# ndpp/ndpp

Hardware: AMD Instinct MI355X
Metric: E_in points*Legendre-orders/sec (free-gas scatter moments) (higher is better)
Workload: dtype f64

## Files before the change

ndpp_amd/csrc/fg_device.h:

```cpp
#pragma once

#include <hip/hip_runtime.h>

#include "fg_pipeline.h"

namespace ndpp {
namespace {

constexpr int kWave = 64;
constexpr int kMuWavesPerSimd = 2;
constexpr int kMuBlocksPerCU = 4 * kMuWavesPerSimd;

struct DevAtomics {
  __device__ static int add(int* p, int v) { return atomicAdd(p, v); }
};

typedef __attribute__((address_space(3))) double lds_f64;
typedef __attribute__((address_space(3))) unsigned lds_u32;

constexpr int mu_stack_fields(int R) { return 2 + 2 * R; }
constexpr int mu_lds_levels(int R) {
  const int budget = (160 * 1024) / kMuBlocksPerCU - 64;
  const int fit = budget / (kWave * (8 * mu_stack_fields(R) + 4));
  return (R == 1 && fit > kStackLdsLevels) ? kStackLdsLevels : fit;
// ... 38 lines not shown
        Xb[r] = lds[o + (2 + r) * kWave];
        Xe[r] = lds[o + (2 + R + r) * kWave];
      }
      m = ldsm[(d - d0) * kWave + lane];
    } else {
      const double* p = (const double*)(gbase + (size_t)(goff + __umul24((unsigned)d, gstride)));
      b = p[0]; w = p[1];
#pragma unroll
      for (int r = 0; r < R; ++r) { Xb[r] = p[2 + r]; Xe[r] = p[2 + R + r]; }
      m = *(const unsigned*)(p + NF);
    }
  }
};

__global__ void fg_prep_kernel(FgBatch B, int level) {
  if (*B.overflow) return;
  const int base = B.lvl_off(level);
  const int nt = B.n_tasks(level);
  for (int t = blockIdx.x * blockDim.x + threadIdx.x; t < nt;
       t += gridDim.x * blockDim.x)
    fg_prep_task(B, level, base, t);
}

template <int R, int LMAX, bool kPath>
__device__ __forceinline__ void mu_wave_loop(const FgBatch& B, int level, int base, int nt,
                                             int* counter, DevMuStack<R>& st) {
  MuLane<R, LMAX> s;
  s.mask = 0;
  const PnConsts pk = make_pn_consts<(R * LMAX <= 12 && LMAX <= 8)>();
  bool active = false, more = true;
  bool counts = true;
  unsigned long long n_k = 0, n_v = 0, n_i = 0, n_o = 0;
  unsigned long long w_it = 0, l_it = 0;
  const int kTaskBlock = nt >= (int)(gridDim.x * 16 * kWave) ? 4 * kWave : kWave;
  int blk_next = 0, blk_end = 0;
  constexpr int kFetchMin = kPath ? 8 : 1;
  auto lanes = [](bool x) -> unsigned long long { return __builtin_amdgcn_ballot_w64(x); };
  for (;;) {
    unsigned long long need = more ? lanes(!active) : 0ull;
    if (kFetchMin > 1 && need && __popcll(need) < kFetchMin && lanes(active)) need = 0;
    if (need) {
      if (blk_next >= blk_end) {
        const int first = __ffsll((long long)need) - 1;
        int b = 0;
        if (threadIdx.x == (unsigned)first) b = atomicAdd(counter, kTaskBlock);
        b = __builtin_amdgcn_readlane(b, first);
        blk_next = b;
        blk_end = (b + kTaskBlock < nt) ? b + kTaskBlock : nt;
        if (b >= nt) more = false;
      }
      if (!active && more) {
        const int rank = __popcll(need & ((1ull << threadIdx.x) - 1ull));
        const int t = blk_next + rank;
        if (t < blk_end) {
          if (kPath) mu_init_split<R, LMAX>(B, level, base, t, s);
          else mu_init<R, LMAX>(B, level, base, t, s);
          active = (s.mask != 0);
          if (kPath) counts = (s.path_bits == 0);
          if (active) mu_tot_zero(s);
        }
      }
      const int taken = __popcll(need);
      blk_next = (blk_next + taken < blk_end) ? blk_next + taken : blk_end;
    }
    const unsigned long long act = lanes(active);
    if (!act && !more) break;
    w_it += 1;
    l_it += (unsigned long long)__popcll(act);
    if (active) {
      if (!mu_step<R, LMAX, DevMuStack<R>, kPath>(B, s, st, pk)) {
        mu_finish(B, s, kPath);
        n_k += 2ull * s.visits + 3;
        n_v += s.visits;
        n_o += s.ovisits;
        n_i += counts ? 1 : 0;
        active = false;
      }
    }
  }
// ... 8 lines not shown
    atomicAdd(&B.stats[kStatMuVisits], n_v);
    atomicAdd(&B.stats[kStatMuIntegrals], n_i);
    atomicAdd(&B.stats[kStatOrderVisits], n_o);
    atomicAdd(&B.stats[kStatWaveIters], w_it);
    atomicAdd(&B.stats[kStatLaneIters], l_it);
  }
}

template <int R, int LMAX>
__global__ __launch_bounds__(kWave, kMuWavesPerSimd) void fg_mu_kernel(FgBatch B, int level, double* gstack, int* counter) {
  constexpr int NF = mu_stack_fields(R), kLevels = mu_lds_levels(R);
  __shared__ double lds[kLevels * NF * kWave];
  __shared__ unsigned ldsm[kLevels * kWave];
  DevMuStack<R> st;
  st.lds = (lds_f64*)lds;
  st.ldsm = (lds_u32*)ldsm;
  st.gbase = (char*)gstack;
  st.goff = (blockIdx.x * kWave + threadIdx.x) * DevMuStack<R>::kRecBytes;
  st.gstride = gridDim.x * kWave * DevMuStack<R>::kRecBytes;
  st.lane = threadIdx.x;
  st.d0 = B.mu_its > kLevels ? B.mu_its - kLevels : 0;

  if (*B.overflow) return;
  const int base = B.lvl_off(level);
  if (B.split_level(level))
    mu_wave_loop<R, LMAX, true>(B, level, base, B.n_mu_tasks(level) * kSplit, counter, st);
  else
    mu_wave_loop<R, LMAX, false>(B, level, base, B.n_mu_tasks(level), counter, st);
}

__global__ void fg_seg_zero_kernel(FgBatch B, int level) {
  if (*B.overflow || !B.split_level(level)) return;
  const size_t n = (size_t)B.n_mu_tasks(level) * kSplit * B.nch();
  for (size_t k = blockIdx.x * (size_t)blockDim.x + threadIdx.x; k < n; k += (size_t)gridDim.x * blockDim.x)
    B.seg[k] = 0.0;
}

__global__ void fg_mu_combine_kernel(FgBatch B, int level) {
  if (*B.overflow || !B.split_level(level)) return;
  const int base = B.lvl_off(level);
  const int nch = B.nch();
  const long tot = (long)B.n_mu_tasks(level) * nch;
  for (long k = blockIdx.x * (long)blockDim.x + threadIdx.x; k < tot; k += (long)gridDim.x * blockDim.x) {
    const int t = (int)(k / nch), ch = (int)(k - (long)t * nch);
    int n, slot;
    fg_task_decode(B, level, base, t, n, slot);
    const unsigned mask = (unsigned)B.node_info[4 * n + 0];
    const int r = ch / B.L, l = ch - r * B.L;
    if (!(mask & chan_bit(r, l))) continue;
    const unsigned gl_rows = B.t_gl ? B.t_gl[B.rec_index(level, base, n, slot)] : 0u;
    if (gl_rows >> r & 1u) continue;
// ... 28 lines not shown
  const int nn = B.lvl_cnt[level];
  for (int i = blockIdx.x * blockDim.x + threadIdx.x; i < nn;
       i += gridDim.x * blockDim.x)
    fg_reduce_node(B, base, i);
}

__global__ void fg_assemble_kernel(FgBatch B) {
  if (*B.overflow) return;
  const int n_calls = B.n_jobs * B.R;
  for (int c = blockIdx.x * blockDim.x + threadIdx.x; c < n_calls;
       c += gridDim.x * blockDim.x)
    fg_assemble_call(B, c);
}

inline int fg_blocks(long n, int threads = 256) {
  long b = (n + threads - 1) / threads;
  return (int)(b < 1 ? 1 : (b > 4096 ? 4096 : b));
}
inline void launch_fg_setup(const FgBatch& B, hipStream_t s) {
  hipLaunchKernelGGL(fg_setup_kernel, dim3(fg_blocks((long)B.n_jobs * B.G)), dim3(256), 0, s, B);
}
inline void launch_fg_prep(const FgBatch& B, int level, hipStream_t s) {
  hipLaunchKernelGGL(fg_prep_kernel, dim3(2048), dim3(256), 0, s, B, level);
}
inline void launch_fg_seg_zero(const FgBatch& B, int level, hipStream_t s) {
  hipLaunchKernelGGL(fg_seg_zero_kernel, dim3(4096), dim3(256), 0, s, B, level);
}
inline void launch_fg_combine(const FgBatch& B, int level, hipStream_t s) {
  hipLaunchKernelGGL(fg_mu_combine_kernel, dim3(2048), dim3(256), 0, s, B, level);
}
inline void launch_fg_node(const FgBatch& B, int level, hipStream_t s) {
  hipLaunchKernelGGL(fg_node_kernel, dim3(2048), dim3(256), 0, s, B, level);
}
inline void launch_fg_reduce(const FgBatch& B, int level, hipStream_t s) {
  hipLaunchKernelGGL(fg_reduce_kernel, dim3(2048), dim3(256), 0, s, B, level);
}
inline void launch_fg_assemble(const FgBatch& B, hipStream_t s) {
  hipLaunchKernelGGL(fg_assemble_kernel, dim3(fg_blocks((long)B.n_jobs * B.R)), dim3(256), 0, s, B);
}

#if NDPP_FAST
template <int R, int LMAX>
__global__ __launch_bounds__(256) void fg_gauss_kernel(FgBatch B, int level) {
  __shared__ int queue[256 / kWave][2 * kWave];
  if (*B.overflow) return;
  const int base = B.lvl_off(level);
// ... 184 lines not shown
```

ndpp_amd/csrc/fg_pipeline.h:

```cpp
#pragma once

#include "ndpp_math.h"

namespace ndpp {
#if NDPP_FAST
inline namespace fast_arith {
#else
inline namespace strict_arith {
#endif

#if NDPP_FAST
constexpr int kMuBlock = 2;
#else
constexpr int kMuBlock = 1;
#endif
constexpr int kSegPerGroup = 5;
constexpr int kMaxLevels = 32;
constexpr int kStackLdsLevels = 8;
constexpr int kMaxRows = 2;
constexpr int kSplitLog2 = 4;
constexpr int kSplit = 1 << kSplitLog2;
constexpr int kRowBits = 16;

enum { kStatKEvals = 0, kStatMuVisits, kStatMuIntegrals, kStatEoutNodes,
       kStatWaveIters, kStatLaneIters, kStatOrderVisits, kStatGaussIntegrals, kNumStats };

NDPP_HD unsigned chan_bit(int r, int l) { return 1u << (r * kRowBits + l); }

struct FgBatch {
  int n_jobs, R, G, L, M;
  double A, kT;
  const double* job_A = nullptr;
  const double* job_kT = nullptr;
  const double* job_ein;
  const int* job_row;
  const double* f_tab;
  const double* e_bins;
  double sab_threshold, brent_thresh, mu_tol, eout_tol;
  int mu_its, eout_its;
  MuGrid grid;
  int ncap;
  double* node_a;
  double* node_b;
  double* node_F;
  double* node_S;
// ... 1 lines not shown
  int tcap;
  double* t_mulo;
  double* t_muhi;
  double* t_X;
  unsigned char* t_gl = nullptr;
  double gl_ratio = 2.0;
  int gl_near = 1;
  double gl_amin = 2.0E-6;
  int gl_cert_depth = 7;
  int gl_cert_depth_near = 8;
  int gl_panels = 16;
  int gl_graded = 8;
  int* lvl_cnt;
  int* next_task;
  int* overflow;
  unsigned long long* stats;
  double* seg = nullptr;
  int split_below = 0;
  const int* order = nullptr;
  const int* mask_rank = nullptr;
  const int* mu_nodes = nullptr;
  double* raw;
  int* t_alias = nullptr;

  NDPP_HD double A_of(int job) const { return job_A ? job_A[job] : A; }
  NDPP_HD double kT_of(int job) const { return job_kT ? job_kT[job] : kT; }
  NDPP_HD int nch() const { return R * L; }
  NDPP_HD int n_trees() const { return n_jobs * G * kSegPerGroup; }
  NDPP_HD int lvl_off(int level) const {
    int o = 0;
    for (int k = 0; k < level; ++k) o += lvl_cnt[k];
    return o;
  }
  NDPP_HD bool split_level(int level) const {
    const int nt = n_mu_tasks(level);
    return seg != nullptr && nt > 0 && nt <= split_below;
  }
  NDPP_HD int tasks_per_node(int level) const { return level == 0 ? 5 : 2; }
  NDPP_HD int n_tasks(int level) const { return lvl_cnt[level] * tasks_per_node(level); }
  NDPP_HD int n_mu_tasks(int level) const {
    return (mu_nodes ? *mu_nodes : lvl_cnt[level]) * tasks_per_node(level);
  }
  NDPP_HD int rec_index(int level, int base, int n, int slot) const {
    return level == 0 ? 5 * n + slot : 2 * (n - base) + (slot == 3 ? 1 : 0);
  }
  NDPP_HD double& F(int slot, int ch, int n) const {
    return node_F[((size_t)(slot * R * L + ch)) * ncap + n];
  }
  NDPP_HD double& S(int ch, int n) const { return node_S[(size_t)ch * ncap + n]; }
  NDPP_HD double& tX(int k, int r, int t) const { return t_X[((size_t)(k * R + r)) * tcap + t]; }
  NDPP_HD unsigned full_mask() const {
    unsigned m = 0;
    for (int r = 0; r < R; ++r) m |= ((1u << L) - 1u) << (r * kRowBits);
    return m;
  }
  NDPP_HD int alias_of(int level, int rec) const { return (level == 0 && t_alias && t_gl) ? t_alias[rec] : -1; }
  NDPP_HD int node_job(int n) const { return node_info[4 * n + 2] & 0x3ffffff; }
  NDPP_HD int node_depth(int n) const { return node_info[4 * n + 2] >> 26; }
};

NDPP_HD void fg_group_layout(const FgBatch& B, int job, int g, double* sa, double* sb, bool* live) {
  const double Ein = B.job_ein[job];
  const double A = B.A_of(job), kT = B.kT_of(job);
  double alphaEin = (A - 1.0) / (A + 1.0);
  alphaEin = alphaEin * alphaEin * Ein;
  double Eout_lo, Eout_hi;
  fg_eout_bounds(A, kT, Ein, Eout_lo, Eout_hi);
  const double eg = B.e_bins[g], eg1 = B.e_bins[g + 1];

  bool on[kSegPerGroup] = {false, false, false, false, false};
  if ((eg < Eout_hi) && (eg1 > Eout_lo)) {
    double Elo = (Eout_lo > eg) ? Eout_lo : eg;
    double Ehi = (Eout_hi < eg1) ? Eout_hi : eg1;
// ... 511 lines not shown
  }
  NDPP_HD void pop(int d, double& b_, double& w_, double* Xb_, double* Xe_, unsigned& m_) const {
    b_ = b[d]; w_ = w[d]; m_ = m[d];
    for (int r = 0; r < R; ++r) { Xb_[r] = Xb[d][r]; Xe_[r] = Xe[d][r]; }
  }
};

NDPP_HD int highest_bit(unsigned x) {
#if defined(__HIP_DEVICE_COMPILE__)
  return 31 - __clz((int)x);
#else
  return 31 - __builtin_clz(x);
#endif
}

NDPP_HD int popcount32(unsigned x) {
#if defined(__HIP_DEVICE_COMPILE__)
  return __popc(x);
#else
  return __builtin_popcount(x);
#endif
}

template <int R, int LMAX>
NDPP_HD void mu_init(const FgBatch& B, int level, int base, int t, MuLane<R, LMAX>& s) {
  int n, slot;
  fg_task_decode(B, level, base, t, n, slot);
  s.node = n;
  s.slot = slot;
  s.mask = (unsigned)B.node_info[4 * n + 0] & MuLane<R, LMAX>::kChanMask;
  s.pending = 0;
  s.depth = 0;
  s.visits = 0;
  s.ovisits = 0;
#pragma unroll
  for (int ch = 0; ch < R * LMAX; ++ch) s.acc[ch] = 0.0;
  s.path_left = 0; s.own_from = 0; s.path_bits = 0; s.own_pending = false; s.slot_path = 0;
  s.task = t;
  s.chans = s.mask;
  if (s.mask == 0) return;
  const int rec = B.rec_index(level, base, n, slot);
  if (B.t_gl) {
    const unsigned rows = B.t_gl[rec];
#pragma unroll
    for (int r = 0; r < R; ++r)
      if (rows >> r & 1u) s.mask &= ~(((1u << kRowBits) - 1u) << (r * kRowBits));
    s.chans = s.mask;
    if (s.mask == 0) return;
  }
  const int job = B.node_job(n);
  const double Ein = B.job_ein[job];
  const double Eout = fg_slot_point(B.node_a[n], B.node_b[n], slot);
  s.q = make_pair(B.A_of(job), B.kT_of(job), Ein, Eout);
  s.f.off = 8u * (unsigned)B.M * (unsigned)B.job_row[(size_t)job * R];
  s.a = B.t_mulo[rec];
  s.b = B.t_muhi[rec];
  double Xa[R];
#pragma unroll
  for (int r = 0; r < R; ++r) {
    Xa[r] = B.tX(0, r, rec);
    s.Xb[r] = B.tX(1, r, rec);
    s.Xc[r] = B.tX(2, r, rec);
  }
  const double h = s.b - s.a;
  s.wp = h / 6.0;
  double Pa[LMAX];
  pn_all<LMAX>(s.a, Pa, make_pn_consts());
#pragma unroll
  for (int r = 0; r < R; ++r)
#pragma unroll
    for (int l = 0; l < LMAX; ++l) s.fa[r * LMAX + l] = Xa[r] * Pa[l];
}

template <int R, int LMAX, class Stack, bool kPath = true>
NDPP_HD bool mu_step(const FgBatch& B, MuLane<R, LMAX>& s, Stack& st, const PnConsts& pk) {
  if (kPath && s.own_pending && s.depth == s.own_from) {
    s.own_pending = false;
#pragma unroll
    for (int ch = 0; ch < R * LMAX; ++ch) s.acc[ch] = 0.0;
    mu_tot_zero(s);
  }
  const double c = 0.5 * (s.a + s.b);
  const double h = s.b - s.a;
  const double d = 0.5 * (s.a + c);
  const double e = 0.5 * (c + s.b);
// ... 183 lines not shown
    s.depth = dj + 1;
    return true;
  }
  return false;
}

template <int R, int LMAX>
NDPP_HD void mu_finish(const FgBatch& B, const MuLane<R, LMAX>& s, bool split = false) {
  const unsigned mask = s.chans;
#pragma unroll
  for (int r = 0; r < R; ++r)
#pragma unroll
    for (int l = 0; l < LMAX; ++l)
      if (mask & chan_bit(r, l)) {
        if (split) {
          if (!s.own_pending)
            B.seg[((size_t)s.task * kSplit + s.slot_path) * B.nch() + r * B.L + l] = s.acc[r * LMAX + l];
          continue;
        }
        B.F(s.slot, r * B.L + l, s.node) = s.tot[r * LMAX + l] + s.acc[r * LMAX + l];
      }
}

template <int R, int LMAX>
NDPP_HD void mu_init_split(const FgBatch& B, int level, int base, int t, MuLane<R, LMAX>& s) {
  const int nt = B.n_mu_tasks(level);
  const int i = t % nt, rank = t / nt;
  mu_init<R, LMAX>(B, level, base, i, s);
  int jp = 0;
  if (s.mask != 0) {
#if NDPP_FAST
    const double pa = s.q.p, qa = s.q.q;
#else
    const double pa = s.q.EpE / s.q.AkT, qa = 2.0 * s.q.s2 / s.q.AkT;
#endif
    const double x = ((pa - fabs(s.q.beta)) / qa - s.a) / (s.b - s.a) * (double)kSplit;
    jp = (x > 0.0) ? (x < (double)(kSplit - 1) ? (int)x : kSplit - 1) : 0;
  }
  int lo = jp - 1, hi = jp, cur = hi;
  for (int k = 0; k <= rank; ++k) {
    if (((k & 1) == 0 && hi < kSplit) || lo < 0) cur = hi++;
    else cur = lo--;
  }
  s.path_left = kSplitLog2;
  s.path_bits = (unsigned)cur;
  s.slot_path = 0;
  int tz = 0;
  while (tz < kSplitLog2 && !(((unsigned)cur >> tz) & 1u)) ++tz;
  s.own_from = kSplitLog2 - tz;
  s.own_pending = (s.own_from != 0);
}

NDPP_HD void fg_mu_combine_task(const FgBatch& B, int level, int base, int t) {
  int n, slot;
  fg_task_decode(B, level, base, t, n, slot);
  const unsigned mask = (unsigned)B.node_info[4 * n + 0];
  if (mask == 0) return;
  const unsigned gl_rows = B.t_gl ? B.t_gl[B.rec_index(level, base, n, slot)] : 0u;
  const int nch = B.nch();
  for (int r = 0; r < B.R; ++r)
    for (int l = 0; l < B.L; ++l)
      if ((mask & chan_bit(r, l)) && !(gl_rows >> r & 1u)) {
        const int ch = r * B.L + l;
        double tot = 0.0;
        for (int j = 0; j < kSplit; ++j) tot = tot + B.seg[((size_t)t * kSplit + j) * nch + ch];
        B.F(slot, ch, n) = tot;
      }
}

struct HostAtomics {
  static int add(int* p, int v) { int o = *p; *p += v; return o; }
};

// ... 108 lines not shown
```

ndpp_amd/csrc/fg_strict_stages.hip:

```cpp
#include <cstring>

#include "../../include/ndpp_hip.h"
#include "fg_device.h"
#include "kernels.h"

#if NDPP_FAST
#error "fg_strict_stages.hip must be compiled with -DNDPP_FAST=0 -ffp-contract=off"
#endif

namespace ndpp {
namespace {

template <class Launch>
int strict_stage(const void* batch, size_t batch_bytes, Launch launch) {
  FgBatch B;
  if (batch_bytes != sizeof(FgBatch)) return fail(NDPP_EDEVICE, "strict stage: batch layout mismatch");
  memcpy(&B, batch, sizeof B);
  launch(B);
  return NDPP_OK;
}

int launch_fg_setup_strict(const void* batch, size_t batch_bytes, hipStream_t s) {
  return strict_stage(batch, batch_bytes, [&](const FgBatch& B) { launch_fg_setup(B, s); });
}
int launch_fg_prep_strict(const void* batch, size_t batch_bytes, int level, hipStream_t s) {
  return strict_stage(batch, batch_bytes, [&](const FgBatch& B) { launch_fg_prep(B, level, s); });
}
int launch_fg_seg_zero_strict(const void* batch, size_t batch_bytes, int level, hipStream_t s) {
  return strict_stage(batch, batch_bytes, [&](const FgBatch& B) { launch_fg_seg_zero(B, level, s); });
}
int launch_fg_mu_strict(const void* batch, size_t batch_bytes, int level, int num_cu,
                        double* gstack, int* counter, hipStream_t s) {
  return strict_stage(batch, batch_bytes,
                      [&](const FgBatch& B) { launch_mu_any(B, level, num_cu, gstack, counter, s); });
}
int launch_fg_combine_strict(const void* batch, size_t batch_bytes, int level, hipStream_t s) {
  return strict_stage(batch, batch_bytes, [&](const FgBatch& B) { launch_fg_combine(B, level, s); });
}
int launch_fg_node_strict(const void* batch, size_t batch_bytes, int level, hipStream_t s) {
  return strict_stage(batch, batch_bytes, [&](const FgBatch& B) { launch_fg_node(B, level, s); });
}
int launch_fg_reduce_strict(const void* batch, size_t batch_bytes, int level, hipStream_t s) {
  return strict_stage(batch, batch_bytes, [&](const FgBatch& B) { launch_fg_reduce(B, level, s); });
}
int launch_fg_assemble_strict(const void* batch, size_t batch_bytes, hipStream_t s) {
  return strict_stage(batch, batch_bytes, [&](const FgBatch& B) { launch_fg_assemble(B, s); });
}

}

const FgStages& fg_strict_stages() {
  static const FgStages table = {launch_fg_setup_strict,  launch_fg_prep_strict,    launch_fg_seg_zero_strict,
                                 launch_fg_mu_strict,     launch_fg_combine_strict, launch_fg_node_strict,
                                 launch_fg_reduce_strict, launch_fg_assemble_strict};
  return table;
}

}
```

ndpp_amd/csrc/kernels.h:

```cpp
#pragma once
#include <hip/hip_runtime.h>

#include <type_traits>

#include "../../include/ndpp_hip.h"

namespace ndpp {

int fail(int code, const char* fmt, ...);

#define NDPP_TRY(expr)                                                        \
  do {                                                                        \
    hipError_t e_ = (expr);                                                   \
    if (e_ != hipSuccess)                                                     \
      return fail(NDPP_EDEVICE, "%s failed: %s (%s:%d)", #expr,               \
                  hipGetErrorString(e_), __FILE__, __LINE__);                 \
  } while (0)

int require_device(const char* who = nullptr);
int check_row_lo(int n_ein, const int* row_lo, int n_rows);
int check_law9_edata(int n_edata, const double* edata);
enum ParamChecks { kCheckOrder = 1, kCheckTab = 2, kCheckFreegas = 4 };
int check_params(const ndpp_params* p, int G, int what, int n_tab = 0);

// ... 24 lines not shown

enum ProfileFamily { kProfFreegasMu = 0, kProfFreegasOther, kProfFile4, kProfFile6Cm, kProfFile6Lab,
                     kProfLaw9, kProfSab, kProfChi, kProfConvert, kNumProfileFamilies };
void profile_add(int family, double ms);
struct GpuSpan {
  hipEvent_t e0 = nullptr, e1 = nullptr;
  hipStream_t s;
  int family;
  explicit GpuSpan(hipStream_t stream = nullptr, int family = -1);
  void end();
  ~GpuSpan();
};

void launch_file4_any(int n, const int* list, int mu_bins, const double* ein,
                      const int* row_lo, const double* w_hi, const double* f_tab,
                      double awr, double Q, int G, int L, const double* e_bins,
                      int rows_per_ein, double* out, hipStream_t s,
                      const int* nuc_of_ein = nullptr, const double* nuc_awr = nullptr,
                      const double* nuc_Q = nullptr);

struct FgStages {
  int (*setup)(const void* batch, size_t bytes, hipStream_t s);
  int (*prep)(const void* batch, size_t bytes, int level, hipStream_t s);
  int (*seg_zero)(const void* batch, size_t bytes, int level, hipStream_t s);
  int (*mu)(const void* batch, size_t bytes, int level, int num_cu, double* gstack, int* counter, hipStream_t s);
  int (*combine)(const void* batch, size_t bytes, int level, hipStream_t s);
  int (*node)(const void* batch, size_t bytes, int level, hipStream_t s);
  int (*reduce)(const void* batch, size_t bytes, int level, hipStream_t s);
  int (*assemble)(const void* batch, size_t bytes, hipStream_t s);
};
const FgStages& fg_strict_stages();

struct DeviceSink {
  virtual ~DeviceSink() = default;
  virtual int consume(const double* out_d, int n, size_t GL) = 0;
};
int elastic_leg_batch_sink(const ndpp_params* p, double A, double kT, double freegas_cutoff, double Q,
                           int n_ein, const double* ein, const int* row_lo, const double* w_hi,
                           int n_rows, const double* f_tab, int G, const double* e_bins, double* out,
                           int* status, DeviceSink* sink);
int file6_batch_sink(const ndpp_params* p, double awr, int frame_cm, int n_ein, const double* ein,
                     const int* row_lo, int n_rows, const double* e_grid, const int* row_ptr,
                     const double* eout, const double* pdf, const int* intt, const double* f, int G,
                     const double* e_bins, int n_tab, double* out, int* status, DeviceSink* sink,
                     const double* f_dev = nullptr);
int law9_batch_sink(const ndpp_params* p, int n_ein, const double* ein, const int* row_lo,
// ... 26 lines not shown
```

ndpp_amd/csrc/ndpp_hip.hip:

```cpp
#include <hip/hip_runtime.h>

#include <algorithm>
#include <chrono>
#include <cmath>
#include <cstdarg>
#include <cstdio>
#include <cstdlib>
#include <cstring>
#include <mutex>
#include <thread>
#include <vector>

#include "../../include/ndpp_hip.h"
#include "dev_util.h"
#include "fg_device.h"
#include "fg_pipeline.h"
#include "kernels.h"

using namespace ndpp;

namespace {

constexpr int kSortMaxMasks = kSortClasses << 11;

// ... 367 lines not shown
  for (double t : tols)
    if (!(t >= 0.0 && t <= 1.7976931348623157e308))
      return fail(NDPP_EINVAL, "tolerances (sab_threshold, brent_mu_thresh, adaptive_*_tol) must be finite and >= 0");
  return NDPP_OK;
}

namespace {

int check_params(const ndpp_params* p, int G) { return ndpp::check_params(p, G, kCheckOrder | kCheckFreegas); }

inline int gs_blocks(long n, int threads = 256) {
  return (int)std::max<long>(1, std::min<long>((n + threads - 1) / threads, 4096));
}

constexpr int kNodesPerCallGuess = 1024;
constexpr int kNumFgContexts = 4;
constexpr int kTwoContextsMinEin = 128;
constexpr int kTwoContextsMaxEin = 15000;
constexpr int kArenaSpareEin = 64;
size_t bytes_per_node(int nch) {
  return sizeof(double) * (2 + 6 * (size_t)nch) + 4 * sizeof(int)
         + 2 * 8 * sizeof(double)
         + 2
         + sizeof(int);
}

struct NucArrays {
  int n_nuc;
  const double *A, *kT, *cutoff, *Q;
  const int* nuc_of_ein;
};

constexpr double kStrictBelowDefault = 0.0;
constexpr double kStrictColdDefault = 1e-4;
constexpr double kStrictRoughDefault = 1e-12;

void arithmetic_switch(int G, double& strict_x, double& strict_cold, double& rough_rho) {
  strict_x = 0.0;
  strict_cold = 0.0;
  rough_rho = -1.0;
#if NDPP_FAST
  strict_x = kStrictBelowDefault;
  if (const char* sx = getenv("NDPP_HIP_STRICT_BELOW")) {
    strict_x = atof(sx);
    if (!(strict_x > 0.0)) { strict_x = 0.0; return; }
  }
// ... 83 lines not shown
    int dev = 0;
    NDPP_TRY(hipGetDevice(&dev));
    NDPP_TRY(hipGetDeviceProperties(&prop, dev));
    g_ws.num_cu = prop.multiProcessorCount;
  }
  pl.num_cu = g_ws.num_cu;
  pl.mu_blocks = g_ws.num_cu * kMuBlocksPerCU;
  pl.mu_threads = (size_t)pl.mu_blocks * kWave;
  if (pl.mu_threads * DevMuStack<2>::kRecBytes >= ((size_t)1 << 24))
    return fail(NDPP_EDEVICE, "%d compute units: the sibling-stack addressing assumes fewer than 4681 workgroups", g_ws.num_cu);
  pl.gstack_doubles = 0;
  for (int R = 1; R <= (pl.joint ? 2 : 1); ++R) {
    const size_t lv = (size_t)std::max(0, p->adaptive_mu_its - (R == 1 ? mu_lds_levels(1) : mu_lds_levels(2)));
    pl.gstack_doubles = std::max(pl.gstack_doubles, lv * ((R == 1 ? mu_stack_fields(1) : mu_stack_fields(2)) + 1) * pl.mu_threads);
  }
  const size_t split_cap = std::min<size_t>((size_t)1 << 22, std::max<size_t>((size_t)n_ein * 128, (size_t)1 << 16));
  pl.split_below = t.split ? (int)std::min<size_t>((size_t)(t.split_x * pl.mu_threads), split_cap) : 0;
  pl.seg_doubles = (size_t)pl.split_below * kSplit * pl.nch;
  pl.ctx_fixed = (pl.seg_doubles + pl.gstack_doubles + 3) * sizeof(double) +
                 sizeof(int) * (((size_t)kSortClasses << L) + 4 * (kMaxLevels + 2) + 128) + 10 * 256;
  pl.fixed = (size_t)n_ein * 3 * sizeof(int) + (size_t)n_rows * sizeof(int) + (1u << 20) +
             sizeof(int) * ((size_t)1 << L) + pl.contexts * pl.ctx_fixed + 4096;
  const size_t node_bytes = bytes_per_node(pl.nch);
  const size_t per_job_bytes = sizeof(double) * (GL + 3) + sizeof(int) * 2 + 16 + sizeof(int) * 25 * (size_t)G;
  const size_t whole = pl.fixed + ((size_t)n_ein + pl.contexts * pl.spare_ein) * pl.nodes_per_ein * node_bytes +
                       (size_t)n_ein * rows_per_ein * per_job_bytes + 4096;
  size_t budget;
  if (g_ws.base && whole <= g_ws.bytes) {
    budget = g_ws.bytes;
    free_b = g_ws.bytes;
  } else {
    NDPP_TRY(hipMemGetInfo(&free_b, &total_b));
    if (g_ws.base) free_b += g_ws.bytes;
    budget = std::min<size_t>((size_t)(free_b * 0.6), (size_t)128 << 30);
  }
  size_t ncap = (budget > pl.fixed ? budget - pl.fixed : 0) /
                (node_bytes + (per_job_bytes * rows_per_ein + pl.nodes_per_ein - 1) / pl.nodes_per_ein);
  ncap = std::min<size_t>(ncap, ((size_t)n_ein + pl.contexts * pl.spare_ein) * pl.nodes_per_ein);
  ncap = std::min<size_t>(ncap, (size_t)0x7fffffff / 5);
  if (t.max_chunk_ein) ncap = std::min<size_t>(ncap, (size_t)t.max_chunk_ein * pl.nodes_per_ein);
  if (ncap < pl.nodes_per_ein)
    return fail(NDPP_ENOMEM, "not enough device memory for one incoming energy (free %zu)", free_b);
  pl.ncap = (long)ncap;
  pl.max_jobs = (long)std::min<size_t>((size_t)n_ein, ncap / pl.nodes_per_ein) * rows_per_ein;
  pl.need = pl.fixed + (size_t)pl.ncap * node_bytes + (size_t)pl.max_jobs * per_job_bytes;
  return NDPP_OK;
}
// ... 80 lines not shown
  if (a.nuc.nuc_of_ein)
    hipLaunchKernelGGL(check_nuc_kernel, grid, block, 0, stream, a.n_ein, a.nuc.nuc_of_ein, a.nuc.n_nuc,
                       h.counters + 4);
  if (look_at_tables)
    hipLaunchKernelGGL(fg_rough_kernel, dim3(std::min(a.n_rows, 4096)), block, 0, stream, a.n_rows, a.p->mu_bins,
                       a.f_tab, t.rough_rho, h.rough);
  hipLaunchKernelGGL(classify_kernel, grid, block, 0, stream, a.n_ein, a.ein, a.cutoff, h.fg_list, h.counters + 0,
                     h.f4_list, h.counters + 1, a.nuc.nuc_of_ein, a.nuc.cutoff, a.out, a.GL(),
                     t.strict_x, t.strict_cold, a.A, a.kT, a.nuc.A, a.nuc.kT, h.fgs_list, h.counters + 5,
                     look_at_tables ? h.rough : nullptr, a.row_lo, a.rows_per_ein, a.n_rows);
  int hc[6];
  NDPP_TRY(hipMemcpyAsync(hc, h.counters, sizeof(hc), hipMemcpyDeviceToHost, stream));
  NDPP_TRY(hipStreamSynchronize(stream));
  if (hc[3]) return fail(NDPP_EINVAL, "row_lo outside [0, n_rows-%d]", a.rows_per_ein);
  if (hc[4]) return fail(NDPP_EINVAL, "nuc_of_ein outside [0, n_nuc)");
  h.n_fast = hc[0], h.n_f4 = hc[1], h.n_strict = hc[5];
  return NDPP_OK;
}

inline const FgBatch& own(const void* batch) { return *static_cast<const FgBatch*>(batch); }
const FgStages kFgOwnStages = {
    [](const void* b, size_t, hipStream_t s) { launch_fg_setup(own(b), s); return 0; },
    [](const void* b, size_t, int level, hipStream_t s) { launch_fg_prep(own(b), level, s); return 0; },
    [](const void* b, size_t, int level, hipStream_t s) { launch_fg_seg_zero(own(b), level, s); return 0; },
    [](const void* b, size_t, int level, int num_cu, double* gstack, int* counter, hipStream_t s) {
      launch_mu_any(own(b), level, num_cu, gstack, counter, s); return 0; },
    [](const void* b, size_t, int level, hipStream_t s) { launch_fg_combine(own(b), level, s); return 0; },
    [](const void* b, size_t, int level, hipStream_t s) { launch_fg_node(own(b), level, s); return 0; },
    [](const void* b, size_t, int level, hipStream_t s) { launch_fg_reduce(own(b), level, s); return 0; },
    [](const void* b, size_t, hipStream_t s) { launch_fg_assemble(own(b), s); return 0; },
};

struct FgCtx {
  FgBatch B;
  Slot sl;
  bool strict;
  const FgStages* stages;
  const int* list;
  int lstride;
  long n, done, chunk_ein, this_ein;
  double *job_ein, *job_A, *job_kT;
  int *job_row, *order;
  bool inflight;
  std::vector<EventPair> walk_ev;
  std::vector<EventPair> gauss_ev;
};
// ... 45 lines not shown
    FgCtx& c = ctx[k];
    if (!side_by_side) cv.p = arena;
    c.sl = h.slot[side_by_side ? k : 0];
    if (side_by_side && k > 0) c.sl.s = ws.aux[k - 1];
    long share = side_by_side ? std::max<long>((long)pl.nodes_per_ein,
                                               (long)((double)ncap * (c.n + pl.spare_ein) /
                                                      (n_all + (long)nctx * pl.spare_ein))) : ncap;
    share = std::min<long>(share, (long)((size_t)(c.n + pl.spare_ein) * pl.nodes_per_ein));
    if (side_by_side) {
      share = std::min(share, cap_left - (long)(nctx - 1 - k) * (long)pl.nodes_per_ein);
      cap_left -= share;
    }
    const long max_jobs = std::min<long>(c.n, share / (long)pl.nodes_per_ein) * a.rows_per_ein;
    FgBatch& B = c.B;
    B = T;
    B.ncap = (int)share;
    B.node_a = cv.take<double>(B.ncap); B.node_b = cv.take<double>(B.ncap);
    B.node_F = cv.take<double>((size_t)5 * pl.nch * B.ncap);
    B.node_S = cv.take<double>((size_t)pl.nch * B.ncap);
    B.node_info = cv.take<int>((size_t)4 * B.ncap);
    B.tcap = 2 * B.ncap;
    B.t_mulo = cv.take<double>(B.tcap); B.t_muhi = cv.take<double>(B.tcap);
    B.t_X = cv.take<double>((size_t)3 * (pl.joint ? 2 : 1) * B.tcap);
    B.t_gl = (gauss_on && !c.strict) ? cv.take<unsigned char>(B.tcap) : nullptr;
    B.t_alias = (t.alias && B.t_gl) ? cv.take<int>((size_t)25 * a.G * max_jobs) : nullptr;
    B.job_ein = c.job_ein = cv.take<double>(max_jobs);
    B.job_row = c.job_row = cv.take<int>(max_jobs);
    c.job_A = cv.take<double>(max_jobs); c.job_kT = cv.take<double>(max_jobs);
    if (a.nuc.nuc_of_ein) { B.job_A = c.job_A; B.job_kT = c.job_kT; }
    B.raw = cv.take<double>((size_t)max_jobs * a.GL());
    c.order = cv.take<int>(B.ncap);
    B.order = t.sort ? c.order : nullptr;
    B.seg = pl.split_below ? c.sl.seg : nullptr;
    B.lvl_cnt = c.sl.lvl_cnt; B.next_task = c.sl.next_task; B.overflow = c.sl.overflow;
    if (cv.p > cv.end)
      return fail(NDPP_ENOMEM, "workspace carve overran (%zu > %zu)",
                  (size_t)(cv.p - ws.base), ws.bytes);
    c.chunk_ein = std::max<long>(1, max_jobs / a.rows_per_ein);
    if (t.max_chunk_ein) c.chunk_ein = std::min<long>(c.chunk_ein, t.max_chunk_ein);
  }
  return NDPP_OK;
}

struct Drain {
  hipStream_t first;
  hipStream_t* more;
// ... 52 lines not shown
    stats->wave_iters = hs[kStatWaveIters];
    stats->lane_iters = hs[kStatLaneIters];
    stats->order_visits = hs[kStatOrderVisits];
    stats->gauss_integrals = hs[kStatGaussIntegrals];
    stats->gauss_ms = gauss_sum_ms;
    for (int k = 0; k < 32; ++k) stats->mu_level_ms[k] = level_ms[k];
    stats->mu_kernel_ms = mu_sum_ms;
    stats->mu_busy_ms = mu_ms;
    stats->mu_kernel_launches = mu_launches;
    stats->contexts = contexts;
    stats->total_ms = ms;
  }
};

int enqueue_chunk(FgCtx& c, const BatchCall& a, const FgTunables& t, const BatchPlan& pl) {
  FgBatch& B = c.B;
  hipStream_t s = c.sl.s;
  const FgStages& st = *c.stages;
  const int rows_per_ein = a.rows_per_ein, GL = a.GL();
  for (;;) {
    c.this_ein = std::min<long>(c.chunk_ein, c.n - c.done);
    B.n_jobs = pl.joint ? (int)c.this_ein : (int)(c.this_ein * rows_per_ein);
    const int ntrees = B.n_trees();
    if ((long)ntrees * kSegPerGroup <= (long)B.tcap && ntrees <= B.ncap) break;
    if (c.chunk_ein <= 1) return fail(NDPP_EOVERFLOW, "arena of %d nodes is too small for one E_in", B.ncap);
    c.chunk_ein = std::max<long>(1, c.chunk_ein / 2);
  }
  const int* lst = c.list + (size_t)c.done * c.lstride;
  NDPP_TRY(hipMemsetAsync(c.sl.lvl_cnt, 0, (kMaxLevels + 2) * sizeof(int), s));
  NDPP_TRY(hipMemsetAsync(c.sl.next_task, 0, 2 * (kMaxLevels + 2) * sizeof(int), s));
  NDPP_TRY(hipMemsetAsync(c.sl.overflow, 0, sizeof(int), s));
  hipLaunchKernelGGL(fg_set_int_kernel, dim3(1), dim3(1), 0, s, c.sl.lvl_cnt, B.n_trees());
  hipLaunchKernelGGL(make_jobs_kernel, dim3(gs_blocks(B.n_jobs)), dim3(256), 0, s, B.n_jobs, rows_per_ein, pl.joint,
                     lst, c.lstride, a.ein, a.row_lo, c.job_ein, c.job_row, a.nuc.nuc_of_ein, a.nuc.A, a.nuc.kT,
                     c.job_A, c.job_kT);
  if (int rc = st.setup(&B, sizeof B, s)) return rc;
  const int nlev = B.eout_its + 1;
  for (int level = 0; level < nlev; ++level) {
    B.mu_nodes = nullptr;
    if (int rc = fg_strict_stages().prep(&B, sizeof B, level, s)) return rc;
    if (B.t_gl) {
      c.gauss_ev.emplace_back();
      NDPP_TRY(c.gauss_ev.back().before.record(s));
      launch_gauss_any(B, level, pl.num_cu, t.gauss_phased, s);
      NDPP_TRY(c.gauss_ev.back().after.record(s));
    }
    if (t.sort) {
      B.mu_nodes = c.sl.mu_nodes;
      NDPP_TRY(hipMemsetAsync(c.sl.mask_hist, 0, sizeof(int) * pl.nb_sort, s));
      hipLaunchKernelGGL(fg_sort_count_kernel, dim3(1024), dim3(256), 0, s, B, level, pl.nb_sort, c.sl.mask_hist);
      hipLaunchKernelGGL(fg_sort_scan_kernel, dim3(1), dim3(256), 0, s, c.sl.mask_hist, pl.nb_sort, c.sl.mu_nodes);
      hipLaunchKernelGGL(fg_sort_scatter_kernel, dim3(1024), dim3(256), 0, s, B, level, pl.nb_sort,
                         c.sl.mask_hist, c.order);
    }
    if (B.seg)
      if (int rc = st.seg_zero(&B, sizeof B, level, s)) return rc;
    c.walk_ev.emplace_back();
    NDPP_TRY(c.walk_ev.back().before.record(s));
    if (int rc = st.mu(&B, sizeof B, level, pl.num_cu, c.sl.gstack, c.sl.next_task + level, s)) return rc;
    NDPP_TRY(c.walk_ev.back().after.record(s));
    if (int rc = st.combine(&B, sizeof B, level, s)) return rc;
    B.mu_nodes = nullptr;
    if (int rc = st.node(&B, sizeof B, level, s)) return rc;
  }
  for (int level = nlev - 1; level >= 0; --level)
    if (int rc = st.reduce(&B, sizeof B, level, s)) return rc;
  if (int rc = st.assemble(&B, sizeof B, s)) return rc;
  if (rows_per_ein == 2)
    hipLaunchKernelGGL(blend_kernel, dim3(gs_blocks(c.this_ein * GL)), dim3(256), 0, s,
                       (int)c.this_ein, lst, c.lstride, B.raw, a.w_hi, GL, a.out);
  else
    hipLaunchKernelGGL(copy_raw_kernel, dim3(gs_blocks(c.this_ein * GL)), dim3(256), 0, s,
                       (int)c.this_ein, lst, c.lstride, B.raw, GL, a.out);
  c.inflight = true;
  return NDPP_OK;
}

// ... 409 lines not shown
```

Baseline: 304,100.

## Precompute per-task mu items in a separate kernel before the walk

```diff
diff --git a/ndpp_amd/csrc/fg_device.h b/ndpp_amd/csrc/fg_device.h
--- a/ndpp_amd/csrc/fg_device.h
+++ b/ndpp_amd/csrc/fg_device.h
@@ -84,8 +84,21 @@
     fg_prep_task(B, level, base, t);
 }
 
+template <int R>
+__global__ void fg_item_kernel(FgBatch B, int level) {
+  if (*B.overflow) return;
+  const int base = B.lvl_off(level);
+  const int nt = B.n_mu_tasks(level);
+  if (nt > B.icap) {
+    if (blockIdx.x == 0 && threadIdx.x == 0) *B.overflow = 1;
+    return;
+  }
+  for (int i = blockIdx.x * blockDim.x + threadIdx.x; i < nt; i += gridDim.x * blockDim.x)
+    fg_item_build<R>(B, level, base, i, i);
+}
+
 template <int R, int LMAX, bool kPath>
-__device__ __forceinline__ void mu_wave_loop(const FgBatch& B, int level, int base, int nt,
+__device__ __forceinline__ void mu_wave_loop(const FgBatch& B, int nt,
                                              int* counter, DevMuStack<R>& st) {
   MuLane<R, LMAX> s;
   s.mask = 0;
@@ -96,7 +109,9 @@
   unsigned long long w_it = 0, l_it = 0;
   const int kTaskBlock = nt >= (int)(gridDim.x * 16 * kWave) ? 4 * kWave : kWave;
   int blk_next = 0, blk_end = 0;
-  constexpr int kFetchMin = kPath ? 8 : 1;
+  const int nti = kPath ? nt >> kSplitLog2 : nt;
+  int blk_first = 0, blk_rank = 0, blk_rem = 0;
+  constexpr int kFetchMin = kPath ? 2 : 1;
   auto lanes = [](bool x) -> unsigned long long { return __builtin_amdgcn_ballot_w64(x); };
   for (;;) {
     unsigned long long need = more ? lanes(!active) : 0ull;
@@ -110,13 +125,27 @@
         blk_next = b;
         blk_end = (b + kTaskBlock < nt) ? b + kTaskBlock : nt;
         if (b >= nt) more = false;
+        if (kPath && more) {
+          blk_first = b;
+          blk_rank = b / nti;
+          blk_rem = b - blk_rank * nti;
+        }
       }
       if (!active && more) {
-        const int rank = __popcll(need & ((1ull << threadIdx.x) - 1ull));
-        const int t = blk_next + rank;
+        const int t = blk_next + __popcll(need & ((1ull << threadIdx.x) - 1ull));
         if (t < blk_end) {
-          if (kPath) mu_init_split<R, LMAX>(B, level, base, t, s);
-          else mu_init<R, LMAX>(B, level, base, t, s);
+          if (kPath) {
+            int i = blk_rem + (t - blk_first), rank = blk_rank;
+            if (nti >= 4 * kWave) {
+              if (i >= nti) { i -= nti; rank += 1; }
+            } else {
+              rank = t / nti;
+              i = t - rank * nti;
+            }
+            mu_init_split<R, LMAX>(B, i, rank, s);
+          } else {
+            mu_init<R, LMAX>(B, t, s);
+          }
           active = (s.mask != 0);
           if (kPath) counts = (s.path_bits == 0);
           if (active) mu_tot_zero(s);
@@ -171,11 +200,10 @@
   st.d0 = B.mu_its > kLevels ? B.mu_its - kLevels : 0;
 
   if (*B.overflow) return;
-  const int base = B.lvl_off(level);
   if (B.split_level(level))
-    mu_wave_loop<R, LMAX, true>(B, level, base, B.n_mu_tasks(level) * kSplit, counter, st);
+    mu_wave_loop<R, LMAX, true>(B, B.n_mu_tasks(level) * kSplit, counter, st);
   else
-    mu_wave_loop<R, LMAX, false>(B, level, base, B.n_mu_tasks(level), counter, st);
+    mu_wave_loop<R, LMAX, false>(B, B.n_mu_tasks(level), counter, st);
 }
 
 __global__ void fg_seg_zero_kernel(FgBatch B, int level) {
@@ -250,6 +278,10 @@
 }
 inline void launch_fg_prep(const FgBatch& B, int level, hipStream_t s) {
   hipLaunchKernelGGL(fg_prep_kernel, dim3(2048), dim3(256), 0, s, B, level);
+}
+inline void launch_fg_item(const FgBatch& B, int level, hipStream_t s) {
+  if (B.R == 2) hipLaunchKernelGGL(fg_item_kernel<2>, dim3(2048), dim3(256), 0, s, B, level);
+  else hipLaunchKernelGGL(fg_item_kernel<1>, dim3(2048), dim3(256), 0, s, B, level);
 }
 inline void launch_fg_seg_zero(const FgBatch& B, int level, hipStream_t s) {
   hipLaunchKernelGGL(fg_seg_zero_kernel, dim3(4096), dim3(256), 0, s, B, level);
diff --git a/ndpp_amd/csrc/fg_pipeline.h b/ndpp_amd/csrc/fg_pipeline.h
--- a/ndpp_amd/csrc/fg_pipeline.h
+++ b/ndpp_amd/csrc/fg_pipeline.h
@@ -21,6 +21,16 @@
 constexpr int kSplitLog2 = 4;
 constexpr int kSplit = 1 << kSplitLog2;
 constexpr int kRowBits = 16;
+constexpr int kItemA = 0, kItemB = 1, kItemXa = 2, kItemXb = kItemXa + kMaxRows, kItemXc = kItemXb + kMaxRows;
+constexpr int kItemPair = kItemXc + kMaxRows;
+constexpr int kItemPairFast = 4, kItemPairStrict = 9;
+constexpr int kItemDoublesFast = kItemPair + kItemPairFast, kItemDoublesStrict = kItemPair + kItemPairStrict;
+#if NDPP_FAST
+constexpr int kItemDoubles = kItemDoublesFast;
+#else
+constexpr int kItemDoubles = kItemDoublesStrict;
+#endif
+enum ItemInt { kItemMask = 0, kItemNodeSlot, kItemOff, kItemJp, kItemInts };
 
 enum { kStatKEvals = 0, kStatMuVisits, kStatMuIntegrals, kStatEoutNodes,
        kStatWaveIters, kStatLaneIters, kStatOrderVisits, kStatGaussIntegrals, kNumStats };
@@ -68,6 +78,9 @@
   const int* mu_nodes = nullptr;
   double* raw;
   int* t_alias = nullptr;
+  int icap = 0;
+  double* it_d = nullptr;
+  int* it_i = nullptr;
 
   NDPP_HD double A_of(int job) const { return job_A ? job_A[job] : A; }
   NDPP_HD double kT_of(int job) const { return job_kT ? job_kT[job] : kT; }
@@ -95,6 +108,8 @@
   }
   NDPP_HD double& S(int ch, int n) const { return node_S[(size_t)ch * ncap + n]; }
   NDPP_HD double& tX(int k, int r, int t) const { return t_X[((size_t)(k * R + r)) * tcap + t]; }
+  NDPP_HD double& itd(int field, int i) const { return it_d[(size_t)field * icap + i]; }
+  NDPP_HD int& iti(int field, int i) const { return it_i[(size_t)field * icap + i]; }
   NDPP_HD unsigned full_mask() const {
     unsigned m = 0;
     for (int r = 0; r < R; ++r) m |= ((1u << L) - 1u) << (r * kRowBits);
@@ -652,13 +667,74 @@
 #endif
 }
 
+NDPP_HD void item_pair_store(const FgBatch& B, int i, const FgPair& q) {
+  int k = kItemPair;
+#if NDPP_FAST
+  B.itd(k++, i) = q.C1; B.itd(k++, i) = q.p; B.itd(k++, i) = q.q; B.itd(k++, i) = q.beta;
+#else
+  B.itd(k++, i) = q.s1; B.itd(k++, i) = q.c2; B.itd(k++, i) = q.kT; B.itd(k++, i) = q.EpE;
+  B.itd(k++, i) = q.s2; B.itd(k++, i) = q.AkT; B.itd(k++, i) = q.beta;
+  B.itd(k++, i) = q.inv_AkT; B.itd(k++, i) = q.inv_kT;
+#endif
+}
+NDPP_HD FgPair item_pair_load(const FgBatch& B, int i) {
+  FgPair q{};
+  int k = kItemPair;
+#if NDPP_FAST
+  q.C1 = B.itd(k++, i); q.p = B.itd(k++, i); q.q = B.itd(k++, i); q.beta = B.itd(k++, i);
+#else
+  q.s1 = B.itd(k++, i); q.c2 = B.itd(k++, i); q.kT = B.itd(k++, i); q.EpE = B.itd(k++, i);
+  q.s2 = B.itd(k++, i); q.AkT = B.itd(k++, i); q.beta = B.itd(k++, i);
+  q.inv_AkT = B.itd(k++, i); q.inv_kT = B.itd(k++, i);
+#endif
+  return q;
+}
+
+template <int R>
+NDPP_HD void fg_item_build(const FgBatch& B, int level, int base, int i, int at) {
+  int n, slot;
+  fg_task_decode(B, level, base, i, n, slot);
+  B.iti(kItemNodeSlot, at) = (int)((unsigned)n * 8u + (unsigned)slot);
+  unsigned mask = (unsigned)B.node_info[4 * n + 0];
+  const int rec = B.rec_index(level, base, n, slot);
+  if (mask != 0 && B.t_gl) {
+    const unsigned rows = B.t_gl[rec];
+#pragma unroll
+    for (int r = 0; r < R; ++r)
+      if (rows >> r & 1u) mask &= ~(((1u << kRowBits) - 1u) << (r * kRowBits));
+  }
+  B.iti(kItemMask, at) = (int)mask;
+  if (mask == 0) return;
+  const int job = B.node_job(n);
+  const double Ein = B.job_ein[job];
+  const double Eout = fg_slot_point(B.node_a[n], B.node_b[n], slot);
+  const FgPair q = make_pair(B.A_of(job), B.kT_of(job), Ein, Eout);
+  item_pair_store(B, at, q);
+  B.iti(kItemOff, at) = (int)(8u * (unsigned)B.M * (unsigned)B.job_row[(size_t)job * R]);
+  const double a = B.t_mulo[rec], b = B.t_muhi[rec];
+  B.itd(kItemA, at) = a;
+  B.itd(kItemB, at) = b;
+#pragma unroll
+  for (int r = 0; r < R; ++r) {
+    B.itd(kItemXa + r, at) = B.tX(0, r, rec);
+    B.itd(kItemXb + r, at) = B.tX(1, r, rec);
+    B.itd(kItemXc + r, at) = B.tX(2, r, rec);
+  }
+#if NDPP_FAST
+  const double pa = q.p, qa = q.q;
+#else
+  const double pa = q.EpE / q.AkT, qa = 2.0 * q.s2 / q.AkT;
+#endif
+  const double x = ((pa - fabs(q.beta)) / qa - a) / (b - a) * (double)kSplit;
+  B.iti(kItemJp, at) = (x > 0.0) ? (x < (double)(kSplit - 1) ? (int)x : kSplit - 1) : 0;
+}
+
 template <int R, int LMAX>
-NDPP_HD void mu_init(const FgBatch& B, int level, int base, int t, MuLane<R, LMAX>& s) {
-  int n, slot;
-  fg_task_decode(B, level, base, t, n, slot);
-  s.node = n;
-  s.slot = slot;
-  s.mask = (unsigned)B.node_info[4 * n + 0] & MuLane<R, LMAX>::kChanMask;
+NDPP_HD void mu_init(const FgBatch& B, int i, MuLane<R, LMAX>& s) {
+  s.mask = (unsigned)B.iti(kItemMask, i) & MuLane<R, LMAX>::kChanMask;
+  const unsigned ns = (unsigned)B.iti(kItemNodeSlot, i);
+  s.node = (int)(ns >> 3);
+  s.slot = (int)(ns & 7u);
   s.pending = 0;
   s.depth = 0;
   s.visits = 0;
@@ -666,31 +742,19 @@
 #pragma unroll
   for (int ch = 0; ch < R * LMAX; ++ch) s.acc[ch] = 0.0;
   s.path_left = 0; s.own_from = 0; s.path_bits = 0; s.own_pending = false; s.slot_path = 0;
-  s.task = t;
+  s.task = i;
   s.chans = s.mask;
   if (s.mask == 0) return;
-  const int rec = B.rec_index(level, base, n, slot);
-  if (B.t_gl) {
-    const unsigned rows = B.t_gl[rec];
-#pragma unroll
-    for (int r = 0; r < R; ++r)
-      if (rows >> r & 1u) s.mask &= ~(((1u << kRowBits) - 1u) << (r * kRowBits));
-    s.chans = s.mask;
-    if (s.mask == 0) return;
-  }
-  const int job = B.node_job(n);
-  const double Ein = B.job_ein[job];
-  const double Eout = fg_slot_point(B.node_a[n], B.node_b[n], slot);
-  s.q = make_pair(B.A_of(job), B.kT_of(job), Ein, Eout);
-  s.f.off = 8u * (unsigned)B.M * (unsigned)B.job_row[(size_t)job * R];
-  s.a = B.t_mulo[rec];
-  s.b = B.t_muhi[rec];
+  s.q = item_pair_load(B, i);
+  s.f.off = (unsigned)B.iti(kItemOff, i);
+  s.a = B.itd(kItemA, i);
+  s.b = B.itd(kItemB, i);
   double Xa[R];
 #pragma unroll
   for (int r = 0; r < R; ++r) {
-    Xa[r] = B.tX(0, r, rec);
-    s.Xb[r] = B.tX(1, r, rec);
-    s.Xc[r] = B.tX(2, r, rec);
+    Xa[r] = B.itd(kItemXa + r, i);
+    s.Xb[r] = B.itd(kItemXb + r, i);
+    s.Xc[r] = B.itd(kItemXc + r, i);
   }
   const double h = s.b - s.a;
   s.wp = h / 6.0;
@@ -920,33 +984,48 @@
       }
 }
 
+NDPP_HD int split_segment(int jp, int rank) {
+  const int both = 2 * (jp < kSplit - jp ? jp : kSplit - jp);
+  if (rank < both) return (rank & 1) ? jp - ((rank + 1) >> 1) : jp + (rank >> 1);
+  return (jp < kSplit - jp) ? rank : kSplit - 1 - rank;
+}
+NDPP_HD int split_own_from(int seg) {
+  const unsigned low = (unsigned)seg | (1u << kSplitLog2);
+  return kSplitLog2 - highest_bit(low & (0u - low));
+}
+
+template <int R, int LMAX>
+NDPP_HD void mu_init_split(const FgBatch& B, int i, int rank, MuLane<R, LMAX>& s) {
+  mu_init<R, LMAX>(B, i, s);
+  const int cur = split_segment(s.mask != 0 ? B.iti(kItemJp, i) : 0, rank);
+  s.path_left = kSplitLog2;
+  s.path_bits = (unsigned)cur;
+  s.slot_path = 0;
+  s.own_from = split_own_from(cur);
+  s.own_pending = (s.own_from != 0);
+}
+
+template <int R, int LMAX>
+NDPP_HD void mu_init(const FgBatch& B, int level, int base, int t, MuLane<R, LMAX>& s) {
+  double d[kItemDoubles];
+  int w[kItemInts];
+  FgBatch one = B;
+  one.it_d = d; one.it_i = w; one.icap = 1;
+  fg_item_build<R>(one, level, base, t, 0);
+  mu_init<R, LMAX>(one, 0, s);
+  s.task = t;
+}
 template <int R, int LMAX>
 NDPP_HD void mu_init_split(const FgBatch& B, int level, int base, int t, MuLane<R, LMAX>& s) {
   const int nt = B.n_mu_tasks(level);
   const int i = t % nt, rank = t / nt;
-  mu_init<R, LMAX>(B, level, base, i, s);
-  int jp = 0;
-  if (s.mask != 0) {
-#if NDPP_FAST
-    const double pa = s.q.p, qa = s.q.q;
-#else
-    const double pa = s.q.EpE / s.q.AkT, qa = 2.0 * s.q.s2 / s.q.AkT;
-#endif
-    const double x = ((pa - fabs(s.q.beta)) / qa - s.a) / (s.b - s.a) * (double)kSplit;
-    jp = (x > 0.0) ? (x < (double)(kSplit - 1) ? (int)x : kSplit - 1) : 0;
-  }
-  int lo = jp - 1, hi = jp, cur = hi;
-  for (int k = 0; k <= rank; ++k) {
-    if (((k & 1) == 0 && hi < kSplit) || lo < 0) cur = hi++;
-    else cur = lo--;
-  }
-  s.path_left = kSplitLog2;
-  s.path_bits = (unsigned)cur;
-  s.slot_path = 0;
-  int tz = 0;
-  while (tz < kSplitLog2 && !(((unsigned)cur >> tz) & 1u)) ++tz;
-  s.own_from = kSplitLog2 - tz;
-  s.own_pending = (s.own_from != 0);
+  double d[kItemDoubles];
+  int w[kItemInts];
+  FgBatch one = B;
+  one.it_d = d; one.it_i = w; one.icap = 1;
+  fg_item_build<R>(one, level, base, i, 0);
+  mu_init_split<R, LMAX>(one, 0, rank, s);
+  s.task = i;
 }
 
 NDPP_HD void fg_mu_combine_task(const FgBatch& B, int level, int base, int t) {
diff --git a/ndpp_amd/csrc/fg_strict_stages.hip b/ndpp_amd/csrc/fg_strict_stages.hip
--- a/ndpp_amd/csrc/fg_strict_stages.hip
+++ b/ndpp_amd/csrc/fg_strict_stages.hip
@@ -26,6 +26,9 @@
 int launch_fg_prep_strict(const void* batch, size_t batch_bytes, int level, hipStream_t s) {
   return strict_stage(batch, batch_bytes, [&](const FgBatch& B) { launch_fg_prep(B, level, s); });
 }
+int launch_fg_item_strict(const void* batch, size_t batch_bytes, int level, hipStream_t s) {
+  return strict_stage(batch, batch_bytes, [&](const FgBatch& B) { launch_fg_item(B, level, s); });
+}
 int launch_fg_seg_zero_strict(const void* batch, size_t batch_bytes, int level, hipStream_t s) {
   return strict_stage(batch, batch_bytes, [&](const FgBatch& B) { launch_fg_seg_zero(B, level, s); });
 }
@@ -50,9 +53,9 @@
 }
 
 const FgStages& fg_strict_stages() {
-  static const FgStages table = {launch_fg_setup_strict,  launch_fg_prep_strict,    launch_fg_seg_zero_strict,
-                                 launch_fg_mu_strict,     launch_fg_combine_strict, launch_fg_node_strict,
-                                 launch_fg_reduce_strict, launch_fg_assemble_strict};
+  static const FgStages table = {launch_fg_setup_strict,    launch_fg_prep_strict,  launch_fg_item_strict,
+                                 launch_fg_seg_zero_strict, launch_fg_mu_strict,    launch_fg_combine_strict,
+                                 launch_fg_node_strict,     launch_fg_reduce_strict, launch_fg_assemble_strict};
   return table;
 }
 
diff --git a/ndpp_amd/csrc/kernels.h b/ndpp_amd/csrc/kernels.h
--- a/ndpp_amd/csrc/kernels.h
+++ b/ndpp_amd/csrc/kernels.h
@@ -70,6 +70,7 @@
 struct FgStages {
   int (*setup)(const void* batch, size_t bytes, hipStream_t s);
   int (*prep)(const void* batch, size_t bytes, int level, hipStream_t s);
+  int (*item)(const void* batch, size_t bytes, int level, hipStream_t s);
   int (*seg_zero)(const void* batch, size_t bytes, int level, hipStream_t s);
   int (*mu)(const void* batch, size_t bytes, int level, int num_cu, double* gstack, int* counter, hipStream_t s);
   int (*combine)(const void* batch, size_t bytes, int level, hipStream_t s);
diff --git a/ndpp_amd/csrc/ndpp_hip.hip b/ndpp_amd/csrc/ndpp_hip.hip
--- a/ndpp_amd/csrc/ndpp_hip.hip
+++ b/ndpp_amd/csrc/ndpp_hip.hip
@@ -413,6 +413,7 @@
   return sizeof(double) * (2 + 6 * (size_t)nch) + 4 * sizeof(int)
          + 2 * 8 * sizeof(double)
          + 2
+         + kItemDoublesStrict * sizeof(double) + kItemInts * sizeof(int)
          + sizeof(int);
 }
 
@@ -542,7 +543,8 @@
   pl.fixed = (size_t)n_ein * 3 * sizeof(int) + (size_t)n_rows * sizeof(int) + (1u << 20) +
              sizeof(int) * ((size_t)1 << L) + pl.contexts * pl.ctx_fixed + 4096;
   const size_t node_bytes = bytes_per_node(pl.nch);
-  const size_t per_job_bytes = sizeof(double) * (GL + 3) + sizeof(int) * 2 + 16 + sizeof(int) * 25 * (size_t)G;
+  const size_t per_job_bytes = sizeof(double) * (GL + 3) + sizeof(int) * 2 + 16 + sizeof(int) * 25 * (size_t)G +
+                               (kItemDoublesStrict * sizeof(double) + kItemInts * sizeof(int)) * 25 * (size_t)G;
   const size_t whole = pl.fixed + ((size_t)n_ein + pl.contexts * pl.spare_ein) * pl.nodes_per_ein * node_bytes +
                        (size_t)n_ein * rows_per_ein * per_job_bytes + 4096;
   size_t budget;
@@ -669,6 +671,7 @@
 const FgStages kFgOwnStages = {
     [](const void* b, size_t, hipStream_t s) { launch_fg_setup(own(b), s); return 0; },
     [](const void* b, size_t, int level, hipStream_t s) { launch_fg_prep(own(b), level, s); return 0; },
+    [](const void* b, size_t, int level, hipStream_t s) { launch_fg_item(own(b), level, s); return 0; },
     [](const void* b, size_t, int level, hipStream_t s) { launch_fg_seg_zero(own(b), level, s); return 0; },
     [](const void* b, size_t, int level, int num_cu, double* gstack, int* counter, hipStream_t s) {
       launch_mu_any(own(b), level, num_cu, gstack, counter, s); return 0; },
@@ -760,6 +763,9 @@
     B.tcap = 2 * B.ncap;
     B.t_mulo = cv.take<double>(B.tcap); B.t_muhi = cv.take<double>(B.tcap);
     B.t_X = cv.take<double>((size_t)3 * (pl.joint ? 2 : 1) * B.tcap);
+    B.icap = (int)std::min<long>(B.tcap, std::max<long>(B.ncap, 5L * kSegPerGroup * a.G * max_jobs));
+    B.it_d = cv.take<double>((size_t)((c.strict || !NDPP_FAST) ? kItemDoublesStrict : kItemDoublesFast) * B.icap);
+    B.it_i = cv.take<int>((size_t)kItemInts * B.icap);
     B.t_gl = (gauss_on && !c.strict) ? cv.take<unsigned char>(B.tcap) : nullptr;
     B.t_alias = (t.alias && B.t_gl) ? cv.take<int>((size_t)25 * a.G * max_jobs) : nullptr;
     B.job_ein = c.job_ein = cv.take<double>(max_jobs);
@@ -858,7 +864,7 @@
     c.this_ein = std::min<long>(c.chunk_ein, c.n - c.done);
     B.n_jobs = pl.joint ? (int)c.this_ein : (int)(c.this_ein * rows_per_ein);
     const int ntrees = B.n_trees();
-    if ((long)ntrees * kSegPerGroup <= (long)B.tcap && ntrees <= B.ncap) break;
+    if ((long)ntrees * kSegPerGroup <= (long)B.icap && ntrees <= B.ncap) break;
     if (c.chunk_ein <= 1) return fail(NDPP_EOVERFLOW, "arena of %d nodes is too small for one E_in", B.ncap);
     c.chunk_ein = std::max<long>(1, c.chunk_ein / 2);
   }
@@ -889,6 +895,7 @@
       hipLaunchKernelGGL(fg_sort_scatter_kernel, dim3(1024), dim3(256), 0, s, B, level, pl.nb_sort,
                          c.sl.mask_hist, c.order);
     }
+    if (int rc = st.item(&B, sizeof B, level, s)) return rc;
     if (B.seg)
       if (int rc = st.seg_zero(&B, sizeof B, level, s)) return rc;
     c.walk_ev.emplace_back();
```

New measurement: 312,800, median of 6. +2.9%, better.
